# NUStatBioinfo/DegNorm

Hardware: AMD Instinct MI355X
Metric: genes/sec (20k genes x 10 samples, 5 iters) (higher is better)
Workload: dtype f64

## Files before the change

degnorm_amd/_lib.py:

```python
import ctypes
import os
import numpy as np

_HERE = os.path.dirname(os.path.abspath(__file__))
LIB_PATH = os.environ.get('DN_LIB_PATH') or os.path.join(_HERE, 'libdegnorm_amd.so')
TRACE_LEN = 48

DN_OK = 0
DN_E_INVALID, DN_E_HIP, DN_E_STATE, DN_E_UNSUPPORTED, DN_E_NO_DEVICE = -1, -2, -3, -4, -5

NMF_RANK_ONE, NMF, NMF_RATIO = 0, 1, 2
STATUS_NAMES = {0: 'ok', -1: 'ArpackError (all-zero matrix)', -2: 'empty minimum (no |K| >= 1e-5)',
                -3: 'ValueError (fewer than 2 rows or columns)', -4: 'ArpackNoConvergence (solver step cap)'}

EXIT_NAMES = ('low_cov', 'zero_sample', 'median', 'no_loop', 'refined', 'refine_fallback', 'not_found_fallback')

_lib = None


class DegnormAmdError(RuntimeError):
    pass


class Params(ctypes.Structure):
# ... 3 lines not shown


def load(build_if_missing=False):
    global _lib
    if _lib is not None:
        return _lib
    if not os.path.exists(LIB_PATH):
        if build_if_missing:
            from . import build
            build.build_library()
        else:
            raise DegnormAmdError('{0} not found: build it with `python -m degnorm_amd.build` '
                                  '(there is no CPU fallback for the NMF-OA path).'.format(LIB_PATH))
    lib = ctypes.CDLL(LIB_PATH)
    c = ctypes
    vp, i32, i64, dbl = c.c_void_p, c.c_int32, c.c_int64, c.c_double
    P = c.POINTER
    lib.dn_version.restype = c.c_char_p
    lib.dn_last_error.restype = c.c_char_p
    lib.dn_device_count.restype = c.c_int
    lib.dn_p_supported.argtypes = [c.c_int]
    lib.dn_create.argtypes = [c.c_int, P(vp)]
    lib.dn_destroy.argtypes = [vp]
    lib.dn_upload_ragged.argtypes = [vp, i64, i32, P(vp), P(i64), i32, i32, P(i64)]
    lib.dn_upload_packed.argtypes = [vp, i64, i32, P(c.c_float), P(i64)]
    lib.dn_set_downsample_hint.argtypes = [vp, i32]
    lib.dn_set_solver_step_cap.argtypes = [vp, i32]
    lib.dn_set_trace_columns.argtypes = [vp, i32]
    lib.dn_ratio_svd_sums.argtypes = [vp, P(dbl), P(dbl), P(i32)]
    lib.dn_baseline_iteration.argtypes = [vp, P(dbl), P(Params), P(i64), P(dbl), P(i32), P(i32)]
    lib.dn_fetch_estimates.argtypes = [vp, P(dbl)]
    lib.dn_outer_begin.argtypes = [vp, P(dbl), i32]
    lib.dn_init_begin.argtypes = [vp, P(dbl)]
    lib.dn_init_partials.argtypes = [vp, P(dbl)]
    lib.dn_outer_begin_scaled.argtypes = [vp, P(dbl), i32]
    lib.dn_outer_partials.argtypes = [vp, P(dbl)]
    lib.dn_outer_apply.argtypes = [vp, P(dbl), P(dbl), i32]
    lib.dn_fetch_outer.argtypes = [vp, P(dbl), P(dbl), P(dbl), P(c.c_uint8)]
    lib.dn_fetch_rows.argtypes = [vp, i64, P(i64), P(dbl), P(i32)]
    lib.dn_fetch_estimates_subset.argtypes = [vp, i64, P(i64), P(dbl)]
    lib.dn_last_kernel_ms.argtypes = [vp]
    lib.dn_last_kernel_ms.restype = dbl
    lib.dn_main_kernel_name.argtypes = [vp]
    lib.dn_main_kernel_name.restype = c.c_char_p
    lib.dn_last_span_ms.argtypes = [vp]
    lib.dn_last_span_ms.restype = dbl
    lib.dn_last_init_ms.argtypes = [vp]
    lib.dn_last_init_ms.restype = dbl
    lib.dn_init_kernel_name.argtypes = [vp]
    lib.dn_init_kernel_name.restype = c.c_char_p
    lib.dn_split_length.argtypes = [vp]
    lib.dn_split_length.restype = i32
    lib.dn_class_lengths.argtypes = [vp, i32, i32, P(i32), P(i32)]
    lib.dn_tiny_length.argtypes = [vp]
    lib.dn_tiny_length.restype = i32
    lib.dn_class_kernel_ms.argtypes = [vp, c.c_int]
    lib.dn_class_kernel_ms.restype = dbl
    lib.dn_class_kernel_name.argtypes = [vp, c.c_int]
    lib.dn_class_kernel_name.restype = c.c_char_p
    lib.dn_synchronize.argtypes = [vp]
    lib.dn_measure_copy_gbps.argtypes = [vp, i64, c.c_int]
    lib.dn_measure_copy_gbps.restype = dbl
    lib.dn_last_rowmax_ms.argtypes = [vp]
    lib.dn_last_rowmax_ms.restype = dbl
    lib.dn_measure_read_gbps.argtypes = [vp, i64, c.c_int]
    lib.dn_measure_read_gbps.restype = dbl
    lib.dn_assemble_coverage.argtypes = [c.c_int, i64, i32, P(i64), P(vp), P(vp), i64, P(i64), i64, P(i32), P(i64), P(i64), P(i32),
                                         P(c.c_float), P(dbl)]
    lib.dn_assemble_last_error.restype = c.c_char_p
    u8 = c.c_uint8
    lib.dn_read_coverage.argtypes = [c.c_int, i32, i64, P(i64), P(i64), P(u8), P(i32), i64, i64, i64, i64, i64, P(i64),
                                     i64, P(i64), P(i32), P(i32), P(i64), P(i64), P(i32), P(i64), i64, P(i64), P(i32),
                                     i64, P(i64), i64, P(i64), P(i64), i64, P(i64), P(i32), P(i64), P(i64), P(dbl)]
    lib.dn_reads_cigar_bounds.argtypes = [c.c_int, i64, P(i64), P(i64), P(u8), i32, P(i32), P(i64), P(i64)]
    lib.dn_reads_last_error.restype = c.c_char_p
    u32 = c.c_uint32
    lib.dn_bam_frame.argtypes = [P(u8), i64, i32, P(i32), P(i64), i64, P(i64), P(i64)]
    lib.dn_bam_rows_create.argtypes = [c.c_int, i32, i32, i32, P(vp)]
    lib.dn_bam_rows_destroy.argtypes = [vp]
    lib.dn_bam_rows_destroy.restype = None
    lib.dn_bam_rows_append.argtypes = [vp, P(u8), i64, P(i64), i64]
    lib.dn_bam_rows_info.argtypes = [vp, P(i64), P(i64), P(i64), P(i32)]
    lib.dn_bam_rows_keys.argtypes = [vp, i32, P(u8)]
    lib.dn_bam_rows_fetch.argtypes = [vp, P(i64), P(i64), P(i32), P(u32), P(i64), P(i32), P(u8)]
    lib.dn_bam_rows_coverage.argtypes = [vp, P(i32), P(i32), i64] + lib.dn_read_coverage.argtypes[8:]
    lib.dn_bam_cigar_bounds.argtypes = [c.c_int, i64, P(i64), P(i64), P(u32), i32, P(i32), P(i64), P(i64)]
    lib.dn_outer_partials_device.argtypes = [vp, P(vp)]
    lib.dn_comm_unique_id.argtypes = [P(c.c_uint8)]
    lib.dn_comm_create.argtypes = [vp, P(c.c_uint8), i32, i32]
    lib.dn_comm_destroy.argtypes = [vp]
    lib.dn_comm_size.argtypes = [vp]
    lib.dn_comm_size.restype = i32
    lib.dn_comm_library.restype = c.c_char_p
    lib.dn_comm_allreduce.argtypes = [vp, P(dbl), i32]
    lib.dn_init_allreduce.argtypes = [vp, P(dbl)]
    lib.dn_outer_allreduce.argtypes = [vp, P(dbl)]
    lib.dn_nmf_f64.argtypes = [vp, i64, i32, P(vp), P(i64), i32, i32, P(dbl), P(dbl), P(dbl), P(i32)]
    lib.dn_baseline_selection_f64.argtypes = [vp, i64, i32, P(vp), P(i64), P(Params), P(i64), P(dbl), P(i32), P(i32), P(dbl)]
    lib.dn_last_f64_ms.argtypes = [vp]
    lib.dn_last_f64_ms.restype = dbl
    _lib = lib
    return lib


def _check(rc):
    if rc == DN_OK:
# ... 281 lines not shown
        return Ks, Es, ests, status

    def baseline_selection_f64(self, mats, nmf_iter=100, bins=20, min_high_coverage=50, downsample_rate=1,
                               skip_baseline_selection=False, ds_start=None, want_est=False):
        keep, ptrs, lengths, p = self._f64_batch(mats)
        n = len(keep)
        prm = Params(int(nmf_iter), int(bins), int(min_high_coverage), int(downsample_rate),
                     int(bool(skip_baseline_selection)), int(bool(want_est)))
        dsp = None
        if ds_start is not None:
            ds_arr = np.ascontiguousarray(ds_start, dtype=np.int64)
            if ds_arr.shape != (n,):
                raise ValueError('ds_start must have one entry per gene')
            dsp = _p(ds_arr, ctypes.c_int64)
        rho = np.zeros((n, p))
        flags = np.zeros(n, dtype=np.int32)
        trace = np.zeros((n, TRACE_LEN), dtype=np.int32)
        est = np.zeros(p * int(lengths.sum())) if want_est else None
        _check(self.lib.dn_baseline_selection_f64(self.h, n, p, ptrs, _p(lengths, ctypes.c_int64), ctypes.byref(prm), dsp,
                                                  _p(rho, ctypes.c_double), _p(flags, ctypes.c_int32), _p(trace, ctypes.c_int32),
                                                  _p(est, ctypes.c_double) if want_est else None))
        ests = None
        if want_est:
            offs = np.concatenate([[0], np.cumsum(lengths)])
            ests = [est[p * offs[k]:p * offs[k + 1]].reshape(p, int(lengths[k])) for k in range(n)]
        return rho, flags.astype(bool), trace, ests

    def last_f64_ms(self):
        return float(self.lib.dn_last_f64_ms(self.h))

    def last_kernel_ms(self):
        return float(self.lib.dn_last_kernel_ms(self.h))

    def last_span_ms(self):
        return float(self.lib.dn_last_span_ms(self.h))

    def last_init_ms(self):
        return float(self.lib.dn_last_init_ms(self.h))

    def init_kernel_name(self):
        return self.lib.dn_init_kernel_name(self.h).decode()

    def main_kernel_name(self):
        return self.lib.dn_main_kernel_name(self.h).decode()

    def split_length(self):
        return int(self.lib.dn_split_length(self.h))

    def class_lengths(self, p, downsample_rate=1):
        a, b = ctypes.c_int32(0), ctypes.c_int32(0)
        _check(self.lib.dn_class_lengths(self.h, int(p), int(downsample_rate), ctypes.byref(a), ctypes.byref(b)))
        return int(a.value), int(b.value)

    def tiny_length(self):
        return int(self.lib.dn_tiny_length(self.h))

    def class_kernel_ms(self, cls):
        return float(self.lib.dn_class_kernel_ms(self.h, int(cls)))

    def class_kernel_name(self, cls):
        return self.lib.dn_class_kernel_name(self.h, int(cls)).decode()

    def measure_copy_gbps(self, nbytes=1 << 30, reps=5):
        return float(self.lib.dn_measure_copy_gbps(self.h, int(nbytes), int(reps)))

    def measure_read_gbps(self, nbytes=1 << 30, reps=5):
        return float(self.lib.dn_measure_read_gbps(self.h, int(nbytes), int(reps)))

    def last_rowmax_ms(self):
        return float(self.lib.dn_last_rowmax_ms(self.h))
```

degnorm_amd/csrc/dn_api.hip:

```cpp
#include "dn_kernels.hpp"
#include "dn_host.hpp"
#include "../../include/degnorm_amd.h"

#include <dlfcn.h>
#include <rccl/rccl.h>

#include <algorithm>
#include <atomic>
#include <cmath>
#include <cstdio>
#include <cstdlib>
#include <cstring>
#include <numeric>
#include <string>
#include <thread>
#include <vector>

#ifndef DN_P_MAX_TEMPLATED
#define DN_P_MAX_TEMPLATED 64
#endif
#define DN_P_2_16(X)  X(2) X(3) X(4) X(5) X(6) X(7) X(8) X(9) X(10) X(11) X(12) X(13) X(14) X(15) X(16)
#define DN_P_17_24(X) X(17) X(18) X(19) X(20) X(21) X(22) X(23) X(24)
#define DN_P_25_32(X) X(25) X(26) X(27) X(28) X(29) X(30) X(31) X(32)
#define DN_P_33_48(X) X(33) X(34) X(35) X(36) X(37) X(38) X(39) X(40) X(41) X(42) X(43) X(44) X(45) X(46) X(47) X(48)
// ... 458 lines not shown
    const int prio[dn_handle_s::NCLS] = {prio_greatest, (prio_least + prio_greatest) / 2, prio_least};
    for (int c = 0; c < dn_handle_s::NCLS; c++) {
        HIP_TRY(h->stream[c].create(hipStreamCreateWithPriority, hipStreamNonBlocking, prio[c]));
        HIP_TRY(h->ev_start[c].create(hipEventCreate));
        HIP_TRY(h->ev_end[c].create(hipEventCreate));
    }
    HIP_TRY(h->ev_ready.create(hipEventCreateWithFlags, hipEventDisableTiming));
    HIP_TRY(h->ev_i0.create(hipEventCreate));
    HIP_TRY(h->ev_i1.create(hipEventCreate));
    return DN_OK;
}

int dn_create(int device, dn_handle *out)
{
    if (!out) return fail(DN_E_INVALID, "dn_create: out is null");
    *out = nullptr;
    int ndev = 0;
    if (hipGetDeviceCount(&ndev) != hipSuccess || ndev <= 0) return fail(DN_E_NO_DEVICE, "no HIP device visible");
    if (device < 0 || device >= ndev) return fail(DN_E_INVALID, "dn_create: device index out of range");
    HIP_TRY(hipSetDevice(device));
    hipDeviceProp_t prop;
    HIP_TRY(hipGetDeviceProperties(&prop, device));
    dn_handle h = new dn_handle_s();
    h->device = device;
    h->n_cus = prop.multiProcessorCount;
    const int rc = create_streams(h);
    if (rc != DN_OK) {
        const std::string msg = g_err;
        (void) dn_destroy(h);
        return fail(rc, msg);
    }
    *out = h;
    return DN_OK;
}

int dn_destroy(dn_handle h)
{
    if (!h) return DN_OK;
    (void) hipSetDevice(h->device);
    if (h->stream[0]) (void) hipStreamSynchronize(h->stream[0]);
    (void) dn_comm_destroy(h);
    delete h;
    return DN_OK;
}

static int size_class(dn_handle h, dn_handle_s::GeneClass &C, int32_t cols)
{
    const int32_t p = h->p;
    int per_cu = C.ks->blocks_per_cu(0);
    if (per_cu < 1) per_cu = 1;
    const int units = std::max(1, C.ks->units);
    int slots = (int) std::min<int64_t>(((int64_t) C.n + units - 1) / units * units, (int64_t) per_cu * h->n_cus * units);
    const int32_t S = (cols + 63) & ~63;
    const int64_t slot_bytes = (int64_t) S * ((int64_t) p * (2 * sizeof(float) + sizeof(double)) + 3 * sizeof(double)) + (int64_t) C.ks->slot_extra_bytes;
    {
        size_t free_b = 0, total_b = 0;
        HIP_TRY(hipMemGetInfo(&free_b, &total_b));
        const int64_t budget = (int64_t) ((free_b + (C.d_ws ? (size_t) C.slot_bytes * (size_t) std::max(C.slots, 1) : 0)) / 3);
        if (slot_bytes > budget) return fail(DN_E_INVALID, "a gene is too long for the device scratch (" + std::to_string(S) + " columns)");
        slots = (int) std::max<int64_t>(units, std::min<int64_t>(slots, budget / slot_bytes / units * units));
    }
    dn::DeviceBuffer<char> ws;
    HIP_TRY(ws.alloc((size_t) slot_bytes * (size_t) std::max(slots, 1)));
    C.d_ws = std::move(ws);
    C.slots = slots; C.S = S; C.slot_bytes = slot_bytes;
    const int64_t lds_per_block = (160 * 1024) / per_cu - (int64_t) C.ks->static_lds_bytes - 256;
    const int64_t ps = p + (p & 1);
    int64_t lcols = lds_per_block > 0 ? lds_per_block / units / (8 * ps) : 0;
    lcols = std::min<int64_t>(lcols, C.S) & ~(int64_t) 1;
    C.lds_cols = (int32_t) lcols;
    C.dyn_lds = (size_t) units * (size_t) lcols * 8 * (size_t) ps;
    return DN_OK;
}

struct CoverageSource {
    const float *packed = nullptr;
    const void *const *genes = nullptr;
    int32_t is_f32 = 0, n_threads = 1;
    std::atomic<int64_t> *bad = nullptr;
};

static void pack_genes(dn_handle h, const CoverageSource &src, int64_t g0, int64_t g1, float *stage)
{
    const int32_t p = h->p;
    const int64_t base = h->goff[g0];
    std::atomic<int64_t> next(g0);
    auto work = [&]() {
        int64_t local_bad = 0;
        for (;;) {
            const int64_t a = next.fetch_add(16);
            if (a >= g1) break;
            const int64_t b = std::min(g1, a + 16);
            for (int64_t g = a; g < b; g++) {
                const int64_t cnt = (int64_t) p * h->glen[g];
                float *dst = stage + (h->goff[g] - base);
                if (src.is_f32) std::memcpy(dst, src.genes[g], sizeof(float) * (size_t) cnt);
                else {
                    const double *s = (const double *) src.genes[g];
                    for (int64_t k = 0; k < cnt; k++) { const float f = (float) s[k]; dst[k] = f; local_bad += ((double) f != s[k]); }
                }
            }
        }
        if (src.bad) *src.bad += local_bad;
    };
    const int nt = (int) std::max<int64_t>(1, std::min<int64_t>(src.n_threads, (g1 - g0 + 15) / 16));
    std::vector<std::thread> th;
    for (int t = 1; t < nt; t++) th.emplace_back(work);
// ... 901 lines not shown
    HIP_TRY(hipMemsetAsync(d_counter, 0, sizeof(int32_t) * 4, h->stream[0]));
    HIP_TRY(hipMemsetAsync(d_trace, 0, sizeof(int32_t) * (size_t) n * dn::TRACE_LEN, h->stream[0]));
    if (d_ds) HIP_TRY(hipMemcpyAsync(d_ds, ds_start, sizeof(int64_t) * (size_t) n, hipMemcpyHostToDevice, h->stream[0]));
    if (est) {
        HIP_TRY(hipMemcpyAsync(d_svoff, svoff.data(), sizeof(int64_t) * (size_t) (n + 1), hipMemcpyHostToDevice, h->stream[0]));
        HIP_TRY(hipMemcpyAsync(d_tg, tg.data(), sizeof(int32_t) * tg.size(), hipMemcpyHostToDevice, h->stream[0]));
        HIP_TRY(hipMemcpyAsync(d_tc, tc.data(), sizeof(int32_t) * tc.size(), hipMemcpyHostToDevice, h->stream[0]));
    }
    HIP_TRY(hipEventRecord(e0, h->stream[0]));
    int lrc = dn::launch_row_max_f64(d_cov, d_goff, d_glen, d_rowmax, (int) n, p,
                                     (int) std::min<int64_t>(n, (int64_t) h->n_cus * 8), h->stream[0]);
    if (lrc != 0) return fail(DN_E_HIP, std::string("k_row_max_f64 launch: ") + hipGetErrorString((hipError_t) lrc));

    dn::IterArgsF64 a;
    std::memset(&a, 0, sizeof(a));
    a.cov = d_cov; a.goff = d_goff; a.glen = d_glen; a.order = d_order; a.counter = d_counter; a.ds_start = d_ds;
    a.rowmax = d_rowmax; a.x16 = nullptr; a.ws = d_ws; a.rho = d_rho; a.flags = d_flags; a.trace = d_trace; a.kfin = d_kfin;
    a.emode = d_emode; a.svec = d_svec; a.svoff = d_svoff; a.slot_bytes = slot_bytes; a.n_genes = (int32_t) n; a.S = S;
    a.lds_cols = 0; a.T = prm->nmf_iter; a.bins = prm->bins; a.min_hc = prm->min_high_coverage; a.rate = prm->downsample_rate;
    a.skip = prm->skip_baseline_selection ? 1 : 0; a.want_est = est ? 1 : 0; a.p = p; a.max_steps = h->max_steps;
    for (int i = 0; i < dn::P_MAX; i++) { a.scale[i] = 1.0; a.inv_scale[i] = 1.0; }
    lrc = dn::launch_baseline_f64(a, grid, h->stream[0]);
    if (lrc != 0) return fail(DN_E_HIP, std::string("k_baseline_gen (float64) launch: ") + hipGetErrorString((hipError_t) lrc));
    if (est) {
        dn::EstArgsF64 e;
        std::memset(&e, 0, sizeof(e));
        e.cov = d_cov; e.goff = d_goff; e.glen = d_glen; e.kfin = d_kfin; e.emode = d_emode; e.svec = d_svec; e.svoff = d_svoff;
        e.out = d_est; e.ooff = nullptr; e.n_genes = (int32_t) n; e.p = p;
        for (int i = 0; i < dn::P_MAX; i++) e.scale[i] = 1.0;
        lrc = dn::launch_est_f64(e, d_tg, d_tc, (int) tg.size(), h->stream[0]);
        if (lrc != 0) return fail(DN_E_HIP, std::string("k_estimates_gen (float64) launch: ") + hipGetErrorString((hipError_t) lrc));
    }
    HIP_TRY(hipEventRecord(e1, h->stream[0]));
    HIP_TRY(hipMemcpyAsync(rho, d_rho, sizeof(double) * (size_t) n * p, hipMemcpyDeviceToHost, h->stream[0]));
    HIP_TRY(hipMemcpyAsync(flags, d_flags, sizeof(int32_t) * (size_t) n, hipMemcpyDeviceToHost, h->stream[0]));
    if (trace) HIP_TRY(hipMemcpyAsync(trace, d_trace, sizeof(int32_t) * (size_t) n * dn::TRACE_LEN, hipMemcpyDeviceToHost, h->stream[0]));
    if (est) HIP_TRY(hipMemcpyAsync(est, d_est, sizeof(double) * (size_t) total, hipMemcpyDeviceToHost, h->stream[0]));
    HIP_TRY(hipStreamSynchronize(h->stream[0]));
    HIP_TRY(hipEventElapsedTime(&h->last_f64_ms, e0, e1));
    return DN_OK;
}

double dn_last_f64_ms(dn_handle h) { return h ? (double) h->last_f64_ms : 0.0; }

double dn_last_kernel_ms(dn_handle h) { return h ? (double) h->last_ms : 0.0; }
double dn_last_init_ms(dn_handle h) { return h ? (double) h->last_init_ms : 0.0; }
double dn_last_span_ms(dn_handle h) { return h ? (double) h->last_span_ms : 0.0; }
double dn_last_rowmax_ms(dn_handle h) { return h ? (double) h->last_rowmax_ms : 0.0; }
const char *dn_init_kernel_name(dn_handle h) { return h ? h->init_name : ""; }
const char *dn_main_kernel_name(dn_handle h) { return (h && h->ks) ? h->ks->baseline_name : ""; }
double dn_class_kernel_ms(dn_handle h, int cls) { return (h && cls >= 0 && cls < dn_handle_s::NCLS) ? (double) h->data.cls[cls].last_ms : 0.0; }
const char *dn_class_kernel_name(dn_handle h, int cls) { return (h && cls >= 0 && cls < dn_handle_s::NCLS && h->data.cls[cls].ks && h->data.cls[cls].n > 0) ? h->data.cls[cls].ks->baseline_name : ""; }
int32_t dn_tiny_length(dn_handle h) { return h ? h->tiny_len : 0; }
int dn_class_lengths(dn_handle h, int32_t p, int32_t downsample_rate, int32_t *split_len, int32_t *tiny_len)
{
    if (!h || !split_len || !tiny_len) return fail(DN_E_INVALID, "dn_class_lengths: null argument");
    const dn::KernelSet *ks = dn::kernel_set_for(p);
    if (!ks) return fail(DN_E_UNSUPPORTED, "no kernels compiled for p = " + std::to_string(p));
    HIP_TRY(hipSetDevice(h->device));
    *split_len = 0; *tiny_len = 0;
    if (downsample_rate > 1 && p >= 8) return DN_OK;
    const dn::KernelSet *pair = nullptr;
    class_lengths(ks, p, *split_len, *tiny_len, pair);
    return DN_OK;
}
int32_t dn_split_length(dn_handle h) { return h ? h->split_len : 0; }
int dn_synchronize(dn_handle h)
{
    if (!h) return fail(DN_E_INVALID, "null handle");
    HIP_TRY(hipSetDevice(h->device));
    HIP_TRY(hipStreamSynchronize(h->stream[0]));
    return DN_OK;
}

}

__global__ __launch_bounds__(256) void k_copy4(const float4 *__restrict__ src, float4 *__restrict__ dst, size_t n4)
{
    for (size_t i = (size_t) blockIdx.x * blockDim.x + threadIdx.x; i < n4; i += (size_t) gridDim.x * blockDim.x) dst[i] = src[i];
}

__global__ __launch_bounds__(256) void k_read4(const float4 *__restrict__ src, float *__restrict__ sink, size_t n4)
{
    float acc = 0.f;
    const size_t stride = (size_t) gridDim.x * blockDim.x;
    size_t i = (size_t) blockIdx.x * blockDim.x + threadIdx.x;
    for (; i + 3 * stride < n4; i += 4 * stride) {
        const float4 a = src[i], b = src[i + stride], c = src[i + 2 * stride], d = src[i + 3 * stride];
        acc += (a.x + a.y + a.z + a.w) + (b.x + b.y + b.z + b.w) + (c.x + c.y + c.z + c.w) + (d.x + d.y + d.z + d.w);
    }
    for (; i < n4; i += stride) { const float4 a = src[i]; acc += a.x + a.y + a.z + a.w; }
    if (acc == 12345.678f) sink[0] = acc;
}

__global__ __launch_bounds__(256) void k_read8nt(const float4 *__restrict__ src, float *__restrict__ sink, size_t n4)
{
    float acc = 0.f;
    const size_t stride = (size_t) gridDim.x * blockDim.x;
    size_t i = (size_t) blockIdx.x * blockDim.x + threadIdx.x;
    for (; i + 7 * stride < n4; i += 8 * stride) {
        typedef float vf4 __attribute__((ext_vector_type(4)));
        vf4 v[8];
#pragma unroll
        for (int k = 0; k < 8; k++) v[k] = __builtin_nontemporal_load(reinterpret_cast<const vf4 *>(src + i + k * stride));
#pragma unroll
        for (int k = 0; k < 8; k++) acc += (v[k].x + v[k].y) + (v[k].z + v[k].w);
// ... 59 lines not shown
```

degnorm_amd/csrc/dn_kernels.hpp:

```cpp
#pragma once
#include <hip/hip_runtime.h>
#include <stdint.h>
#include <type_traits>
#include "dn_reduce.hpp"
#include "dn_dpp_ops.hpp"

#ifdef DN_MARKS
#define DN_MARK(name) asm volatile("; DN_MARK " name)
#else
#define DN_MARK(name)
#endif

namespace dn {

constexpr int TRACE_LEN = 48;
constexpr int MAX_BINS = 64;
constexpr int P_MAX = 64;

enum { EXIT_LOW_COV = 0, EXIT_ZERO_SAMPLE = 1, EXIT_MEDIAN = 2, EXIT_NO_LOOP = 3,
       EXIT_REFINED = 4, EXIT_REFINE_FALLBACK = 5, EXIT_NOT_FOUND_FALLBACK = 6 };
enum { LOOP_NATURAL = 0, LOOP_PERFECT = 1, LOOP_VALUE_ERROR = 2, LOOP_ZERO_ROWSUM = 3, LOOP_MIN_BINS = 4,
       LOOP_NOT_ENTERED = 5 };
enum { ST_OK = 0, ST_ARPACK = -1, ST_EMPTY_MIN = -2, ST_VALUE_ERROR = -3,
       ST_NO_CONVERGENCE = -4 };
// ... 962 lines not shown

template <int PS>
__device__ __forceinline__ void lds_col_read(const double *col, double (&a)[PS])
{
#pragma unroll
    for (int i = 0; i < PS; i += 2) { const double2 v = *reinterpret_cast<const double2 *>(col + i); a[i] = v.x; a[i + 1] = v.y; }
}
template <int PS>
__device__ __forceinline__ void lds_col_write(double *col, const double (&a)[PS])
{
#pragma unroll
    for (int i = 0; i < PS; i += 2) *reinterpret_cast<double2 *>(col + i) = make_double2(a[i], a[i + 1]);
}

typedef float dn_f4 __attribute__((ext_vector_type(4)));
typedef float dn_f2 __attribute__((ext_vector_type(2)));
typedef dn_f4 dn_f4u __attribute__((aligned(4)));
typedef dn_f2 dn_f2u __attribute__((aligned(4)));
typedef const dn_f4u __attribute__((address_space(1))) *gF4_cptr;
typedef const dn_f2u __attribute__((address_space(1))) *gF2_cptr;

template <int P>
__device__ __forceinline__ void load_x(gF_cptr Fb, int k, float (&x)[P])
{
    gF_cptr col = Fb + (size_t) k * P;
#pragma unroll
    for (int i = 0; i + 4 <= P; i += 4) {
        const dn_f4 v = *(gF4_cptr) (col + i);
        x[i] = v.x; x[i + 1] = v.y; x[i + 2] = v.z; x[i + 3] = v.w;
    }
    if constexpr ((P & 3) >= 2) {
        const dn_f2 v = *(gF2_cptr) (col + (P & ~3));
        x[P & ~3] = v.x; x[(P & ~3) + 1] = v.y;
    }
    if constexpr (P & 1) x[P - 1] = col[P - 1];
}

template <int P>
__device__ __forceinline__ void load_f(gF_cptr Fb, int k, const double (&inv)[P], double (&f)[P])
{
    float x[P];
    load_x<P>(Fb, k, x);
#pragma unroll
    for (int i = 0; i < P; i++) f[i] = (double) x[i] * inv[i];
}

template <int P, bool RAW>
__device__ __forceinline__ void pass_counts(const float (&x)[P], const double (&inv)[P], double (&f)[P])
{
#pragma unroll
    for (int i = 0; i < P; i++) f[i] = RAW ? (double) x[i] : (double) x[i] * inv[i];
}

template <int P>
__device__ __forceinline__ gdouble_ptr spill_ptr(gdouble_ptr Lg, int k)
{
    return Lg + ((size_t) (k >> 6) * (64 * P) + (size_t) (k & 63));
}

template <int P, int NT>
__device__ __forceinline__ int mg_core(gF_cptr Fb, gdouble_ptr Lg, double *lam, int n, int nL, int T,
                                       double (&u)[P], double &theta, int &steps, int maxs, bool &noconv)
{
    constexpr int W = NT / 64;
    constexpr int NG = P * (P + 1) / 2;
    constexpr int PS = P + (P & 1);
    constexpr int TR = Smem<P, NT>::MG_TR, STR = Smem<P, NT>::MG_STR;
    constexpr int NTILE = TR * (TR + 1) / 2;
    Smem<P, NT> &sm = g_sm;
    const int tid = DN_TIDX, lane = lane_id(), w = wave_id();
    const int nLe = (n < nL) ? n : nL;
    double *stage = &sm.stage[w * 16 * STR];
    double *uv = &sm.eigv[w * 128], *vv = uv + 64;
    const double *invp = g_gs.inv;
    for (int e = lane; e < 16 * STR; e += 64) stage[e] = 0.0;
    uv[lane] = lane < P ? 1.0 / sqrt((double) P) : 0.0;
    vv[lane] = 0.0;
    wave_fence();
    const int oi = lane & 15, okq = lane >> 4;
    dn_double4 acc[NTILE];

    auto feed = [&](const double (&a)[PS], bool valid) {
#pragma unroll
        for (int cq = 0; cq < 4; cq++) {
            if ((lane >> 4) == cq) {
                double *dst = stage + (lane & 15) * STR;
#pragma unroll
                for (int i = 0; i < PS; i += 2) *reinterpret_cast<double2 *>(dst + i) = make_double2(valid ? a[i] : 0.0, valid ? a[i + 1] : 0.0);
            }
            wave_fence();
#pragma unroll
            for (int g = 0; g < 4; g++) {
                double x[TR];
#pragma unroll
                for (int tr = 0; tr < TR; tr++) x[tr] = stage[(4 * g + okq) * STR + 16 * tr + oi];
                int tix = 0;
#pragma unroll
                for (int t1 = 0; t1 < TR; t1++)
#pragma unroll
                    for (int t2 = 0; t2 <= t1; t2++, tix++)
                        acc[tix] = __builtin_amdgcn_mfma_f64_16x16x4f64(x[t1], x[t2], acc[tix], 0, 0, 0);
            }
            wave_fence();
        }
    };

    const double c = 1.0 / sqrt((double) T);
    auto pass = [&](bool cold, int t) {
#pragma unroll
        for (int i = 0; i < NTILE; i++) acc[i] = dn_double4{0.0, 0.0, 0.0, 0.0};
        const int wb = w * 64;
        const int steps_l = wb < nLe ? (nLe - wb + NT - 1) / NT : 0;
        const int steps_s = nL + wb < n ? (n - nL - wb + NT - 1) / NT : 0;
#pragma clang loop unroll(disable)
        for (int j = 0; j < steps_l; j++) {
            const int k = tid + j * NT;
            const bool valid = k < nLe;
            double a[PS];
#pragma unroll
            for (int i = 0; i < PS; i++) a[i] = 0.0;
            if (valid) {
                float xr[P];
                load_x<P>(Fb, k, xr);
                if (cold) {
#pragma unroll
                    for (int i = 0; i < P; i++) a[i] = (double) xr[i] * invp[i];
                } else {
                    double al[PS], aa[P];
                    lds_col_read<PS>(lam + (size_t) k * PS, al);
#pragma unroll
                    for (int i = 0; i < P; i++) aa[i] = al[i];
                    col_update_lds<P>(xr, invp, aa, uv, c);
#pragma unroll
                    for (int i = 0; i < P; i++) a[i] = aa[i];
                }
                lds_col_write<PS>(lam + (size_t) k * PS, a);
            }
            feed(a, valid);
        }
#pragma clang loop unroll(disable)
        for (int j = 0; j < steps_s; j++) {
            const int k = nL + tid + j * NT;
            const bool valid = k < n;
            double a[PS];
#pragma unroll
            for (int i = 0; i < PS; i++) a[i] = 0.0;
            if (valid) {
                float xr[P];
                double aa[P];
                load_x<P>(Fb, k, xr);
                if (cold || t == 0) {
#pragma unroll
                    for (int i = 0; i < P; i++) aa[i] = (double) xr[i] * invp[i];
                } else {
#pragma unroll
                    for (int i = 0; i < P; i++) aa[i] = *(spill_ptr<P>(Lg, k) + i * 64);
                }
                if (!cold) {
                    col_update_lds<P>(xr, invp, aa, uv, c);
#pragma unroll
                    for (int i = 0; i < P; i++) *(spill_ptr<P>(Lg, k) + i * 64) = aa[i];
                }
#pragma unroll
                for (int i = 0; i < P; i++) a[i] = aa[i];
            }
            feed(a, valid);
        }
        {
            double *dst = (W > 1) ? sm.xw[w] : sm.tot;
            int tix = 0;
#pragma unroll
            for (int t1 = 0; t1 < TR; t1++)
#pragma unroll
                for (int t2 = 0; t2 <= t1; t2++, tix++)
#pragma unroll
                    for (int r = 0; r < 4; r++) {
                        const int row = 16 * t1 + okq + 4 * r, col = 16 * t2 + oi;
                        if (row < P && col <= row) dst[row * (row + 1) / 2 + col] = acc[tix][r];
                    }
        }
        if constexpr (W > 1) {
            dn_sync();
            for (int e = tid; e < NG; e += NT) {
                double tsum = sm.xw[0][e];
#pragma unroll
                for (int ww = 1; ww < W; ww++) tsum += sm.xw[ww][e];
                sm.tot[e] = tsum;
            }
        }
        dn_sync();
    };

    pass(true, 0);
    {
        const double tr = wave_allsum(lane < P ? sm.tot[lane * (lane + 1) / 2 + lane] : 0.0);
        if (!(tr > 0.0)) return ST_ARPACK;
    }
    { const int r = top_eig_rows_lds<P>(sm.tot, uv, vv, theta, maxs); steps += r; noconv = noconv || r > maxs; }
    bool cold_every_solve;
    {
        double um = lane < P ? uv[lane] : 1.0;
#pragma unroll
        for (int o = 32; o >= 1; o >>= 1) um = fmin(um, __shfl_xor(um, o));
        cold_every_solve = __builtin_amdgcn_readfirstlane((int) (um < WARM_START_MIN_COMPONENT)) != 0;
    }
#pragma clang loop unroll(disable)
    for (int t = 0; t < T; t++) {
        pass(false, t);
        int r;
        if (!cold_every_solve) r = top_eig_rows_lds<P>(sm.tot, uv, vv, theta, maxs);
        else {
            unsigned long long todo = P >= 64 ? ~0ull : ((1ull << P) - 1ull);
            double bul = 0.0, bth = -1.0;
            int sum = 0;
            bool capped = false;
// ... 227 lines not shown
        }
        block_sum_lds<NQ, P, NT, gram_t, false, Q * CH>(Gq, g_sm);
    });
    {
        double tr = 0.0;
#pragma unroll
        for (int i = 0; i < P; i++) tr += sm.tot[i * (i + 1) / 2 + i];
        if (!(tr > 0.0)) { if (tid == 0) g_gs.status = ST_ARPACK; dn_sync(); return; }
    }
    Solver<P> solver;
    {
        double tr = 0.0;
#pragma unroll
        for (int i = 0; i < P; i++) tr += sm.tot[i * (i + 1) / 2 + i];
        solver.cold(tr, u);
    }
    {
        const int r = SAFE ? solve_by_blocks<P>(solver, sm.tot, Smem<P, NT>::ZSLOT, u, theta, maxs)
                           : solver.run(sm.tot, Smem<P, NT>::ZSLOT, u, theta, T == 0, maxs, true);
        steps += r; noconv = noconv || r > maxs;
    }
    const double c = 1.0 / sqrt((double) T);
    auto pass_u = [&]() {
        if constexpr (RAW) {
            const int k = Solver<P>::row_of_lane() < P ? Solver<P>::row_of_lane() : P - 1;
            const double vt = solver.iterate_of_row() * g_gs.inv[k], vh = solver.iterate_of_row() * g_gs.scl[k];
#pragma unroll
            for (int i = 0; i < P; i++) { ud[i] = Solver<P>::bcast_component(vt, i); ur[i] = Solver<P>::bcast_component(vh, i); }
        } else {
#pragma unroll
            for (int i = 0; i < P; i++) { u[i] = uniform(u[i]); ud[i] = u[i]; ur[i] = u[i]; }
        }
    };
    pass_u();

    static_for<0, RT>([&](auto rc) {
        constexpr int R = decltype(rc)::value;
        const int k = tid + R * NT;
        if (k < n) {
            float xf[P];
            double f[P];
            load_x<P>(Fb, k, xf);
            pass_counts<P, RAW>(xf, inv, f);
            rt_write<P, CS * R>(f);
            if constexpr (X16) rt_write_counts<P, CS * R + 2 * P>(xf);
        }
    });
    for (int k = NR + tid; k < nLe; k += NT) {
        double f[P], a[PS];
        { float xf[P]; load_x<P>(Fb, k, xf); pass_counts<P, RAW>(xf, inv, f); }
#pragma unroll
        for (int i = 0; i < PS; i++) a[i] = i < P ? f[i] : 0.0;
        lds_col_write<PS>(lam + (size_t) (k - NR) * PS, a);
    }
#ifdef DN_STAMP
    stamp[3] += __builtin_amdgcn_s_memtime() - t_cold0;
#endif
    constexpr bool G0 = FULL && ONCHIP && SW == 1;
    constexpr bool SQ = Solver<P>::SQUARE && SW == 1 && !SAFE;
#pragma clang loop unroll(disable)
    for (int t = 0; t < T; t++) {
        DN_MARK("iter_begin");
        if constexpr (!G0) {
#pragma unroll
            for (int i = 0; i < CH; i++) G[i] = 0.0;
        }
        DN_MARK("zeroed");
        { DN_T0();
        const int dir = (t & 1) ? -1 : 1;

        auto reg_tier = [&]() {
            if constexpr (RT > 0 && X16) {
                auto column = [&](auto rc) {
                    constexpr int R = decltype(rc)::value;
                    double f[P], a[P];
                    rt_read_counts<P, CS * R + 2 * P>(f);
                    if constexpr (!RAW) {
#pragma unroll
                        for (int i = 0; i < P; i++) f[i] *= inv[i];
                    }
                    rt_read<P, CS * R>(a);
                    col_update<P>(f, a, ud, ur, c);
                    if constexpr (G0 && R == 0) gram_set_range<P, 0, CH>(G, a); else gram_add_range<P, 0, CH>(G, a);
                    rt_write<P, CS * R>(a);
                };
                if constexpr (FULL) {
                    static_for<0, RT>([&](auto rc) { column(rc); __builtin_amdgcn_sched_barrier(0); });
                } else {
                    static_for<0, RT>([&](auto rc) {
                        constexpr int R = decltype(rc)::value;
                        if (tid + R * NT < n) column(rc);
                    });
                }
            } else if constexpr (RT > 0) {
                float xq[P];
                if (tid < n) load_x<P>(Fb, tid, xq);
                static_for<0, RT>([&](auto rc) {
                    constexpr int R = decltype(rc)::value;
                    const int k = tid + R * NT;
                    if (k < n) {
                        double f[P], a[P];
                        pass_counts<P, RAW>(xq, inv, f);
                        if constexpr (R + 1 < RT) load_x<P>(Fb, k + NT < n ? k + NT : k, xq);
                        rt_read<P, CS * R>(a);
                        col_update<P>(f, a, ud, ur, c);
                        gram_add_range<P, 0, CH>(G, a);
                        rt_write<P, CS * R>(a);
                    }
                });
            }
        };
        auto lds_tier = [&]() {
            const int first = NR + tid;
            const int cnt = first < nLe ? (nLe - first + NT - 1) / NT : 0;
            const int step = dir * NT;
            int k = dir > 0 ? first : first + (cnt - 1) * NT;
            float xq[P];
            if (cnt > 0) load_x<P>(Fb, k, xq);
#pragma clang loop unroll(disable)
            for (int j = 0; j < cnt; j++, k += step) {
                double f[P], a[PS];
                lds_col_read<PS>(lam + (size_t) (k - NR) * PS, a);
                pass_counts<P, RAW>(xq, inv, f);
                load_x<P>(Fb, j + 1 < cnt ? k + step : k, xq);
                double aa[P];
#pragma unroll
                for (int i = 0; i < P; i++) aa[i] = a[i];
                col_update<P>(f, aa, ud, ur, c);
                gram_add_range<P, 0, CH>(G, aa);
#pragma unroll
                for (int i = 0; i < P; i++) a[i] = aa[i];
                lds_col_write<PS>(lam + (size_t) (k - NR) * PS, a);
            }
        };
        auto spill_tier = [&]() {
            if constexpr (ONCHIP) return;
            const int first = kS0 + tid;
            const int cnt = first < n ? (n - first + NT - 1) / NT : 0;
            const int step = dir * NT;
            int k = dir > 0 ? first : first + (cnt - 1) * NT;
            float xn[P];
            double an[P];
            if (cnt > 0) {
                int kq = k;
                asm volatile("" : "+v"(kq));
                load_x<P>(Fb, kq, xn);
                if (t > 0) {
#pragma unroll
                    for (int i = 0; i < P; i++) an[i] = *(spill_ptr<P>(Lg, kq) + i * 64);
                }
            }
#pragma clang loop unroll(disable)
            for (int j = 0; j < cnt; j++, k += step) {
                double f[P], a[P];
                pass_counts<P, RAW>(xn, inv, f);
#pragma unroll
                for (int i = 0; i < P; i++) a[i] = t > 0 ? an[i] : f[i];
                if (j + 1 < cnt) {
                    load_x<P>(Fb, k + step, xn);
                    if (t > 0) {
#pragma unroll
                        for (int i = 0; i < P; i++) an[i] = *(spill_ptr<P>(Lg, k + step) + i * 64);
                    }
                }
                col_update<P>(f, a, ud, ur, c);
                gram_add_range<P, 0, CH>(G, a);
#pragma unroll
                for (int i = 0; i < P; i++) *(spill_ptr<P>(Lg, k) + i * 64) = a[i];
            }
        };
#if defined(DN_STAMP) && defined(DN_EXP_TIER)
#define DN_TIER(id, call) do { if (DN_EXP_TIER == id) { const long long tt_ = __builtin_amdgcn_s_memtime(); call; stamp[0] += __builtin_amdgcn_s_memtime() - tt_; } else { call; } } while (0)
#else
#define DN_TIER(id, call) call
#endif
        if constexpr (G0) { DN_MARK("reg_tier"); DN_TIER(1, reg_tier()); DN_MARK("lds_tier"); DN_TIER(2, lds_tier()); }
        else if (dir > 0) { DN_MARK("reg_tier"); DN_TIER(1, reg_tier()); DN_MARK("lds_tier"); DN_TIER(2, lds_tier()); DN_MARK("spill_tier"); DN_TIER(3, spill_tier()); }
        else { DN_MARK("spill_tier_b"); DN_TIER(3, spill_tier()); DN_MARK("lds_tier_b"); DN_TIER(2, lds_tier()); DN_MARK("reg_tier_b"); DN_TIER(1, reg_tier()); }
        DN_MARK("pass_end");
#if !(defined(DN_STAMP) && defined(DN_EXP_TIER))
        DN_T1(0);
#endif
        }
        { DN_T0(); block_sum_lds<CH, P, NT, gram_t, Solver<P>::SHIFTED, 0, RAW, SQ>(G, sm, solver.shift(), solver.scale(), t & 1); DN_T1(1); }
        DN_MARK("reduced");
        static_for<1, SW>([&](auto qc) {
            constexpr int Q = decltype(qc)::value;
            constexpr int NQ = (NG - Q * CH) < CH ? (NG - Q * CH) : CH;
            gram_t Gq[NQ];
#pragma unroll
            for (int i = 0; i < NQ; i++) Gq[i] = 0.0;
            static_assert(SW == 1 || RT == 0, "the later sweeps do not read the register tier");
#pragma clang loop unroll(disable)
            for (int k = NR + tid; k < nLe; k += NT) {
                double a[PS], aa[P];
                lds_col_read<PS>(lam + (size_t) (k - NR) * PS, a);
#pragma unroll
                for (int i = 0; i < P; i++) aa[i] = a[i];
                gram_add_range<P, Q * CH, NQ>(Gq, aa);
            }
#pragma clang loop unroll(disable)
            for (int k = kS0 + tid; k < n; k += NT) {
                double aa[P];
#pragma unroll
                for (int i = 0; i < P; i++) aa[i] = *(spill_ptr<P>(Lg, k) + i * 64);
                gram_add_range<P, Q * CH, NQ>(Gq, aa);
            }
            block_sum_lds<NQ, P, NT, gram_t, Solver<P>::SHIFTED, Q * CH>(Gq, g_sm, solver.shift());
        });
        { DN_T0();
        double u_unused[P];
        double (&us_)[P] = RAW ? u_unused : u;
        const int r = SAFE ? solve_by_blocks<P>(solver, sm.tot, Smem<P, NT>::ZSLOT, us_, theta, maxs)
                           : solver.template run<SQ>(sm.tot, Smem<P, NT>::ZSLOT, us_, theta, t == T - 1, maxs, false,
                                                     sm.sq + wave_id() * Smem<P, NT>::SQ_LEN);
        steps += r; noconv = noconv || r > maxs;
        pass_u();
        DN_MARK("solved");
        DN_T1(2);
        }
    }
    if constexpr (SQ && NT > 64) dn_sync();
    if constexpr (RAW) {
#pragma unroll
        for (int i = 0; i < P; i++) u[i] = Solver<P>::bcast_component(solver.iterate_of_row(), i);
    }
    }

#ifdef DN_STAMP
    const long long t_fin0 = __builtin_amdgcn_s_memtime();
#endif
    double invf[P];
#pragma unroll
    for (int i = 0; i < P; i++) invf[i] = RAW ? uniform(g_gs.inv[i]) : inv[i];
    double acc[2 * P + 1];
#pragma unroll
    for (int i = 0; i < 2 * P + 1; i++) acc[i] = 0.0;
    auto fin = [&](int k, const double (&f)[P], const double (&l_)[P]) {
        double s, r, l0[P];
#pragma unroll
        for (int i = 0; i < P; i++) l0[i] = RAW ? l_[i] * invf[i] : l_[i];
        col_final<P>(f, l0, u, first, acc, s, r);
        rs[k] = r;
        if (first) sv[k] = s;
    };
    static_for<0, RT>([&](auto rc) {
        constexpr int R = decltype(rc)::value;
        const int k = tid + R * NT;
        if (k < n) {
            double f[P], l[P];
            if constexpr (X16) {
                rt_read_counts<P, CS * R + 2 * P>(f);
#pragma unroll
                for (int i = 0; i < P; i++) f[i] *= invf[i];
            } else load_f<P>(Fb, k, invf, f);
            rt_read<P, CS * R>(l);
            fin(k, f, l);
        }
    });
    float xqf[P];
    if (NR + tid < n) load_x<P>(Fb, NR + tid, xqf);
#pragma clang loop unroll(disable)
    for (int k = NR + tid; k < n; k += NT) {
        double f[P], l[P];
#pragma unroll
        for (int i = 0; i < P; i++) f[i] = (double) xqf[i] * invf[i];
        load_x<P>(Fb, k + NT < n ? k + NT : k, xqf);
        if (k < nLe) {
            double al[PS];
            lds_col_read<PS>(lam + (size_t) (k - NR) * PS, al);
#pragma unroll
            for (int i = 0; i < P; i++) l[i] = al[i];
        } else {
#pragma unroll
            for (int i = 0; i < P; i++) l[i] = *(spill_ptr<P>(Lg, k) + i * 64);
        }
        fin(k, f, l);
    }
    block_sum_lds<2 * P + 1, P, NT, double>(acc, sm);
    for (int e = tid; e < 2 * P + 1; e += NT) g_gs.sums[e] = sm.tot[e];
    if (tid == 0) {
#pragma unroll
        for (int i = 0; i < P; i++) g_gs.u[i] = u[i];
        g_gs.theta = theta;
        g_gs.steps += steps;
        g_gs.status = noconv ? ST_NO_CONVERGENCE : ST_OK;
#ifdef DN_STAMP
        g_gs.stamp[0] += stamp[0]; g_gs.stamp[1] += stamp[1]; g_gs.stamp[2] += stamp[2];
        g_gs.stamp[4] += __builtin_amdgcn_s_memtime() - t_fin0; g_gs.stamp[5] += stamp[3];
#endif
    }
    dn_sync();
}

template <int P, int NT, bool SAFE = false>
__device__ __attribute__((noinline)) void nmf_call(const float *Fb_, double *Lg_, double *rs_, double *sv_, double *rtsave_,
                                                   int n, int S, int nL, int T, int first_i, int x16_i)
{
    constexpr int NSAVE = DN_REG_TIER ? rt_regs_used<P>() : 0;
    int *rtsave = reinterpret_cast<int *>(uniform_ptr(rtsave_));
#ifdef DN_STAMP
    const long long t_call0 = __builtin_amdgcn_s_memtime();
#endif
    const int n_u = __builtin_amdgcn_readfirstlane(n);
    const int need = DN_REG_TIER ? ((n_u + NT - 1) / NT) * rt_col_regs<P, true>() : 0;
    rt_save<NSAVE, NT>(rtsave, need);
    if constexpr (SAFE) {
        nmf_body<P, NT, false, false, false, true>(Fb_, Lg_, rs_, sv_, n, S, nL, T, first_i);
    } else if (DN_REG_TIER && __builtin_amdgcn_readfirstlane(x16_i) != 0) {
        constexpr bool X = DN_REG_TIER != 0;
        const int nL_u = __builtin_amdgcn_readfirstlane(nL);
        if (X && n_u >= rt_cols<P, X>() * NT && n_u <= rt_cols<P, X>() * NT + nL_u)
            nmf_body<P, NT, X, X, X>(Fb_, Lg_, rs_, sv_, n, S, nL, T, first_i);
        else if (X && n_u >= rt_cols<P, X>() * NT) nmf_body<P, NT, X, X>(Fb_, Lg_, rs_, sv_, n, S, nL, T, first_i);
        else nmf_body<P, NT, X, false>(Fb_, Lg_, rs_, sv_, n, S, nL, T, first_i);
    } else nmf_body<P, NT, false>(Fb_, Lg_, rs_, sv_, n, S, nL, T, first_i);
    rt_restore<NSAVE, NT>(rtsave, need);
#ifdef DN_STAMP
    if (DN_TIDX == 0) g_gs.stamp[3] += __builtin_amdgcn_s_memtime() - t_call0;
#endif
}


template <int P> __device__ __forceinline__ double lds_max(const double *v)
{ double m = v[0];
#pragma unroll
  for (int i = 1; i < P; i++) { const double t = v[i]; m = t > m ? t : m; } return m; }
template <int P> __device__ __forceinline__ double lds_min(const double *v)
{ double m = v[0];
#pragma unroll
  for (int i = 1; i < P; i++) { const double t = v[i]; m = t < m ? t : m; } return m; }

template <int P, int NT>
__global__ __launch_bounds__(NT * DN_UNITS, DN_KERNEL_WAVES) void k_baseline(IterArgs A)
{
    constexpr int W = NT / 64;
    Smem<P, NT> &sm = g_sm;
    GeneState<P> &gs = g_gs;
    const int tid = DN_TIDX, lane = lane_id(), w = wave_id();
    const int S = A.S;
    const int nL = A.lds_cols;
    char *slot = A.ws + ((size_t) blockIdx.x * DN_UNITS + DN_UNIT) * A.slot_bytes;
    float *Fs = reinterpret_cast<float *>(slot);
    float *Fb = Fs + (size_t) P * S;
    double *Lg = reinterpret_cast<double *>(Fb + (size_t) P * S);
    double *sv = Lg + (size_t) P * S;
    double *rs = sv + S;
    double *rtsave = rs + 2 * (size_t) S;
    DN_RT_CLAIM();
    if (tid < P) { gs.inv[tid] = A.inv_scale[tid]; gs.scl[tid] = 1.0 / A.inv_scale[tid]; }
    if (tid == 0) gs.max_steps = A.max_steps > 0 ? A.max_steps : EIG_MAX_STEPS_DEFAULT;
    if constexpr (P <= 16) { for (int t = tid; t < W * Smem<P, NT>::SQ_LEN; t += NT) sm.sq[t] = 0.0; }
    for (int t = tid; t < Smem<P, NT>::NX; t += NT) {
        bool diag = false;
        int ra = 0, rb = 0;
#pragma unroll
        for (int i = 0; i < P; i++) {
            diag = diag || (t == i * (i + 1) / 2 + i);
            if (t >= i * (i + 1) / 2) { ra = i; rb = t - i * (i + 1) / 2; }
        }
        if constexpr (P <= 16) sm.sqi[t] = (t < P * (P + 1) / 2) ? (ra * Smem<P, NT>::SQ_STR + rb) | ((rb * Smem<P, NT>::SQ_STR + ra) << 16) : 0;
        if constexpr (raw_units<P>())
            sm.dsel[t] = (t < P * (P + 1) / 2) ? (diag ? -1.0 : 1.0) * A.inv_scale[ra] * A.inv_scale[rb < P ? rb : 0] : 0.0;
        else sm.dsel[t] = diag ? 1.0 : 0.0;
        if (t == Smem<P, NT>::ZSLOT) sm.tot[t] = 0.0;
    }

    for (;;) {
        if (tid == 0) sm.gene = atomicAdd(A.counter, 1);
        dn_sync();
        const int q = sm.gene;
        dn_sync();
        if (q >= A.n_genes) break;
        const int g = A.order[q];
        const int L = A.glen[g];
        const float *x = A.cov + A.goff[g];

        int n0 = 0, n_calls = 0, n_drops = 0, exit_code = EXIT_LOW_COV, loop_reason = LOOP_NOT_ENTERED;
        int status = ST_OK, flag = 0, emode = EM_INPUT;
        long long sum_cols = 0;
#ifdef DN_STAMP
        const long long t_gene0 = __builtin_amdgcn_s_memtime();
        long long t_ret = 0, t_book = 0;
#endif
        int32_t *tr = A.trace + (size_t) g * TRACE_LEN;
        if (tid < P) { gs.rho[tid] = 0.0; gs.K[tid] = 0.0; gs.us[tid] = 0.0; }
        if (tid == 0) { gs.steps = 0; gs.stamp[0] = gs.stamp[1] = gs.stamp[2] = gs.stamp[3] = gs.stamp[4] = gs.stamp[5] = 0; }

        double thr;
        int x16;
        {
            const float *rmx = A.rowmax + (size_t) g * P;
            double gmax = (double) rmx[0] / A.scale[0];
#pragma unroll
            for (int i = 1; i < P; i++) { const double v = (double) rmx[i] / A.scale[i]; gmax = v > gmax ? v : gmax; }
            thr = 0.1 * gmax;
            x16 = A.x16[g];
        }

// ... 419 lines not shown
```

include/degnorm_amd.h:

```cpp
#ifndef DEGNORM_AMD_H
#define DEGNORM_AMD_H

#include <stdint.h>

#ifdef __cplusplus
extern "C" {
#endif

#define DN_OK                 0
#define DN_E_INVALID         -1
#define DN_E_HIP             -2
#define DN_E_STATE           -3
#define DN_E_UNSUPPORTED     -4
#define DN_E_NO_DEVICE       -5

#define DN_TRACE_LEN          48

typedef struct dn_handle_s *dn_handle;

typedef struct {
    int32_t nmf_iter;
    int32_t bins;
    int32_t min_high_coverage;
    int32_t downsample_rate;
// ... 66 lines not shown

#define DN_READS_MAX_SEG      32
int  dn_read_coverage(int device, int32_t paired, int64_t n_rows, const int64_t *pos, const int64_t *cigar_off,
                      const uint8_t *cigar, const int32_t *pair_id, int64_t n_pair_ids,
                      int64_t chrom_len, int64_t keep_lo, int64_t keep_hi,
                      int64_t n_exon, const int64_t *exon_iv,
                      int64_t n_groups, const int64_t *group_iv, const int32_t *group_gene_off,
                      const int32_t *ol_gene, const int64_t *ol_gene_start0, const int64_t *ol_cov_off,
                      const int32_t *ol_exon_off, const int64_t *ol_exon_bounds,
                      int64_t n_iso, const int64_t *iso_iv, const int32_t *iso_gene,
                      int64_t n_iso_union, const int64_t *iso_union,
                      int64_t n_genes, int64_t *counts, int64_t *ol_cov,
                      int64_t csr_cap, int64_t *nnz, int32_t *csr_idx, int64_t *csr_val,
                      int64_t *n_isolated_reads, double *device_ms);
int  dn_reads_cigar_bounds(int device, int64_t n, const int64_t *pos, const int64_t *cigar_off, const uint8_t *cigar,
                           int32_t max_seg, int32_t *nseg, int64_t *bounds, int64_t *end_pos);
const char *dn_reads_last_error(void);

typedef struct dn_bam_rows_s *dn_bam_rows;
int  dn_bam_frame(const uint8_t *buf, int64_t n_bytes, int32_t tid, int32_t *last_pos, int64_t *rec_off, int64_t cap,
                  int64_t *n_rec, int64_t *consumed);
int  dn_bam_rows_create(int device, int32_t tid, int32_t unique_alignment, int32_t paired, dn_bam_rows *out);
void dn_bam_rows_destroy(dn_bam_rows h);
int  dn_bam_rows_append(dn_bam_rows h, const uint8_t *window, int64_t n_bytes, const int64_t *rec_off, int64_t n_rec);
int  dn_bam_rows_info(dn_bam_rows h, int64_t *n_rows, int64_t *n_ops, int64_t *n_name_bytes, int32_t *max_key_len);
int  dn_bam_rows_keys(dn_bam_rows h, int32_t width, uint8_t *keys);
int  dn_bam_rows_fetch(dn_bam_rows h, int64_t *pos, int64_t *op_beg, int32_t *n_op, uint32_t *ops, int64_t *name_beg,
                       int32_t *name_len, uint8_t *names);
int  dn_bam_rows_coverage(dn_bam_rows h, const int32_t *order, const int32_t *pair_id, int64_t n_pair_ids,
                          int64_t chrom_len, int64_t keep_lo, int64_t keep_hi,
                          int64_t n_exon, const int64_t *exon_iv,
                          int64_t n_groups, const int64_t *group_iv, const int32_t *group_gene_off,
                          const int32_t *ol_gene, const int64_t *ol_gene_start0, const int64_t *ol_cov_off,
                          const int32_t *ol_exon_off, const int64_t *ol_exon_bounds,
                          int64_t n_iso, const int64_t *iso_iv, const int32_t *iso_gene,
                          int64_t n_iso_union, const int64_t *iso_union,
                          int64_t n_genes, int64_t *counts, int64_t *ol_cov,
                          int64_t csr_cap, int64_t *nnz, int32_t *csr_idx, int64_t *csr_val,
                          int64_t *n_isolated_reads, double *device_ms);
int  dn_bam_cigar_bounds(int device, int64_t n, const int64_t *pos, const int64_t *op_off, const uint32_t *ops,
                         int32_t max_seg, int32_t *nseg, int64_t *bounds, int64_t *end_pos);

double dn_last_kernel_ms(dn_handle h);
const char *dn_main_kernel_name(dn_handle h);
double dn_last_init_ms(dn_handle h);
double dn_last_rowmax_ms(dn_handle h);
const char *dn_init_kernel_name(dn_handle h);
int32_t dn_split_length(dn_handle h);
int  dn_class_lengths(dn_handle h, int32_t p, int32_t downsample_rate, int32_t *split_len, int32_t *tiny_len);
int32_t dn_tiny_length(dn_handle h);
double dn_class_kernel_ms(dn_handle h, int cls);
double dn_last_span_ms(dn_handle h);
const char *dn_class_kernel_name(dn_handle h, int cls);
int  dn_synchronize(dn_handle h);
double dn_measure_copy_gbps(dn_handle h, int64_t bytes, int reps);
double dn_measure_read_gbps(dn_handle h, int64_t bytes, int reps);

#ifdef __cplusplus
}
#endif
#endif
```

Baseline: 15220.

## Pair-interleave global spill columns for 128-bit loads and prefill spill tier

Changes the global-memory spill layout for per-column lambda values from one double per row-stride to pairs of doubles (padded to an even P), so each column is read and written with 16-byte vector accesses through a shared base pointer with constant offsets. The cold init pass now writes initial spill values, which lets the spill tier loop drop its t==0 branching and always prefetch the next column with clamped indices, restructured as a do-while. It also adds a diagnostic API that reports register/LDS tier column counts. The cost is padding memory for odd P and an extra initial write pass over spilled columns.

```diff
diff --git a/degnorm_amd/_lib.py b/degnorm_amd/_lib.py
--- a/degnorm_amd/_lib.py
+++ b/degnorm_amd/_lib.py
@@ -79,6 +79,7 @@
     lib.dn_split_length.argtypes = [vp]
     lib.dn_split_length.restype = i32
     lib.dn_class_lengths.argtypes = [vp, i32, i32, P(i32), P(i32)]
+    lib.dn_class_tier_cols.argtypes = [vp, c.c_int, P(i32), P(i32)]
     lib.dn_tiny_length.argtypes = [vp]
     lib.dn_tiny_length.restype = i32
     lib.dn_class_kernel_ms.argtypes = [vp, c.c_int]
@@ -466,6 +467,11 @@
         _check(self.lib.dn_class_lengths(self.h, int(p), int(downsample_rate), ctypes.byref(a), ctypes.byref(b)))
         return int(a.value), int(b.value)
 
+    def class_tier_cols(self, cls):
+        a, b = ctypes.c_int32(0), ctypes.c_int32(0)
+        _check(self.lib.dn_class_tier_cols(self.h, int(cls), ctypes.byref(a), ctypes.byref(b)))
+        return int(a.value), int(b.value)
+
     def tiny_length(self):
         return int(self.lib.dn_tiny_length(self.h))
 
diff --git a/degnorm_amd/csrc/dn_api.hip b/degnorm_amd/csrc/dn_api.hip
--- a/degnorm_amd/csrc/dn_api.hip
+++ b/degnorm_amd/csrc/dn_api.hip
@@ -534,7 +534,8 @@
     const int units = std::max(1, C.ks->units);
     int slots = (int) std::min<int64_t>(((int64_t) C.n + units - 1) / units * units, (int64_t) per_cu * h->n_cus * units);
     const int32_t S = (cols + 63) & ~63;
-    const int64_t slot_bytes = (int64_t) S * ((int64_t) p * (2 * sizeof(float) + sizeof(double)) + 3 * sizeof(double)) + (int64_t) C.ks->slot_extra_bytes;
+    const int64_t slot_bytes = (int64_t) S * ((int64_t) p * 2 * sizeof(float) + (int64_t) (p + (p & 1)) * sizeof(double) + 3 * sizeof(double)) +
+                               (int64_t) C.ks->slot_extra_bytes;
     {
         size_t free_b = 0, total_b = 0;
         HIP_TRY(hipMemGetInfo(&free_b, &total_b));
@@ -1542,6 +1543,15 @@
 double dn_class_kernel_ms(dn_handle h, int cls) { return (h && cls >= 0 && cls < dn_handle_s::NCLS) ? (double) h->data.cls[cls].last_ms : 0.0; }
 const char *dn_class_kernel_name(dn_handle h, int cls) { return (h && cls >= 0 && cls < dn_handle_s::NCLS && h->data.cls[cls].ks && h->data.cls[cls].n > 0) ? h->data.cls[cls].ks->baseline_name : ""; }
 int32_t dn_tiny_length(dn_handle h) { return h ? h->tiny_len : 0; }
+int dn_class_tier_cols(dn_handle h, int cls, int32_t *reg_cols, int32_t *lds_cols)
+{
+    if (!h || cls < 0 || cls >= dn_handle_s::NCLS || !reg_cols || !lds_cols) return fail(DN_E_INVALID, "dn_class_tier_cols: bad argument");
+    const auto &C = h->data.cls[cls];
+    const bool live = C.ks && C.n > 0;
+    *reg_cols = live ? C.ks->reg_tier_cols : 0;
+    *lds_cols = live ? C.lds_cols : 0;
+    return DN_OK;
+}
 int dn_class_lengths(dn_handle h, int32_t p, int32_t downsample_rate, int32_t *split_len, int32_t *tiny_len)
 {
     if (!h || !split_len || !tiny_len) return fail(DN_E_INVALID, "dn_class_lengths: null argument");
diff --git a/degnorm_amd/csrc/dn_kernels.hpp b/degnorm_amd/csrc/dn_kernels.hpp
--- a/degnorm_amd/csrc/dn_kernels.hpp
+++ b/degnorm_amd/csrc/dn_kernels.hpp
@@ -1038,10 +1038,32 @@
     for (int i = 0; i < P; i++) f[i] = RAW ? (double) x[i] : (double) x[i] * inv[i];
 }
 
+typedef double dn_d2 __attribute__((ext_vector_type(2)));
+typedef dn_d2 __attribute__((address_space(1))) *gd2_ptr;
+template <int P> constexpr int spill_mid() { return (P + (P & 1)) / 4; }
 template <int P>
-__device__ __forceinline__ gdouble_ptr spill_ptr(gdouble_ptr Lg, int k)
-{
-    return Lg + ((size_t) (k >> 6) * (64 * P) + (size_t) (k & 63));
+__device__ __forceinline__ gd2_ptr spill_col(gdouble_ptr Lg, int k)
+{
+    constexpr int PS = P + (P & 1);
+    gd2_ptr col = (gd2_ptr) (Lg + ((size_t) (k >> 6) * (64 * PS) + (size_t) (k & 63) * 2)) + spill_mid<P>() * 64;
+    asm volatile("" : "+v"(col));
+    return col;
+}
+template <int P>
+__device__ __forceinline__ void spill_col_read(gd2_ptr col, double (&a)[P])
+{
+#pragma unroll
+    for (int q = 0; q < (P + 1) / 2; q++) {
+        const dn_d2 v = col[(q - spill_mid<P>()) * 64];
+        a[2 * q] = v.x;
+        if (2 * q + 1 < P) a[2 * q + 1] = v.y;
+    }
+}
+template <int P>
+__device__ __forceinline__ void spill_col_write(gd2_ptr col, const double (&a)[P])
+{
+#pragma unroll
+    for (int q = 0; q < (P + 1) / 2; q++) col[(q - spill_mid<P>()) * 64] = dn_d2{a[2 * q], 2 * q + 1 < P ? a[2 * q + 1 < P ? 2 * q + 1 : 2 * q] : 0.0};
 }
 
 template <int P, int NT>
@@ -1135,18 +1157,15 @@
                 float xr[P];
                 double aa[P];
                 load_x<P>(Fb, k, xr);
-                if (cold || t == 0) {
+                const gd2_ptr col = spill_col<P>(Lg, k);
+                if (cold) {
 #pragma unroll
                     for (int i = 0; i < P; i++) aa[i] = (double) xr[i] * invp[i];
                 } else {
-#pragma unroll
-                    for (int i = 0; i < P; i++) aa[i] = *(spill_ptr<P>(Lg, k) + i * 64);
+                    spill_col_read<P>(col, aa);
+                    col_update_lds<P>(xr, invp, aa, uv, c);
                 }
-                if (!cold) {
-                    col_update_lds<P>(xr, invp, aa, uv, c);
-#pragma unroll
-                    for (int i = 0; i < P; i++) *(spill_ptr<P>(Lg, k) + i * 64) = aa[i];
-                }
+                spill_col_write<P>(col, aa);
 #pragma unroll
                 for (int i = 0; i < P; i++) a[i] = aa[i];
             }
@@ -1480,6 +1499,13 @@
 #pragma unroll
         for (int i = 0; i < PS; i++) a[i] = i < P ? f[i] : 0.0;
         lds_col_write<PS>(lam + (size_t) (k - NR) * PS, a);
+    }
+    if constexpr (!ONCHIP) {
+        for (int k = kS0 + tid; k < n; k += NT) {
+            double f[P];
+            { float xf[P]; load_x<P>(Fb, k, xf); pass_counts<P, RAW>(xf, inv, f); }
+            spill_col_write<P>(spill_col<P>(Lg, k), f);
+        }
     }
 #ifdef DN_STAMP
     stamp[3] += __builtin_amdgcn_s_memtime() - t_cold0;
@@ -1563,39 +1589,34 @@
         };
         auto spill_tier = [&]() {
             if constexpr (ONCHIP) return;
-            const int first = kS0 + tid;
-            const int cnt = first < n ? (n - first + NT - 1) / NT : 0;
+            int tq = tid;
+            asm volatile("" : "+v"(tq));
+            const int first = kS0 + tq;
+            if (first >= n) return;
             const int step = dir * NT;
-            int k = dir > 0 ? first : first + (cnt - 1) * NT;
+            const int last = first + (n - 1 - first) / NT * NT;
+            int k = dir > 0 ? first : last;
+            const int kend = dir > 0 ? last : first;
             float xn[P];
             double an[P];
-            if (cnt > 0) {
-                int kq = k;
-                asm volatile("" : "+v"(kq));
-                load_x<P>(Fb, kq, xn);
-                if (t > 0) {
-#pragma unroll
-                    for (int i = 0; i < P; i++) an[i] = *(spill_ptr<P>(Lg, kq) + i * 64);
-                }
-            }
+            load_x<P>(Fb, k, xn);
+            spill_col_read<P>(spill_col<P>(Lg, k), an);
+            bool more;
 #pragma clang loop unroll(disable)
-            for (int j = 0; j < cnt; j++, k += step) {
+            do {
                 double f[P], a[P];
                 pass_counts<P, RAW>(xn, inv, f);
 #pragma unroll
-                for (int i = 0; i < P; i++) a[i] = t > 0 ? an[i] : f[i];
-                if (j + 1 < cnt) {
-                    load_x<P>(Fb, k + step, xn);
-                    if (t > 0) {
-#pragma unroll
-                        for (int i = 0; i < P; i++) an[i] = *(spill_ptr<P>(Lg, k + step) + i * 64);
-                    }
-                }
+                for (int i = 0; i < P; i++) a[i] = an[i];
+                const int kn = dir > 0 ? min(k + step, kend) : max(k + step, kend);
+                load_x<P>(Fb, kn, xn);
+                spill_col_read<P>(spill_col<P>(Lg, kn), an);
                 col_update<P>(f, a, ud, ur, c);
                 gram_add_range<P, 0, CH>(G, a);
-#pragma unroll
-                for (int i = 0; i < P; i++) *(spill_ptr<P>(Lg, k) + i * 64) = a[i];
-            }
+                spill_col_write<P>(spill_col<P>(Lg, k), a);
+                more = k != kend;
+                k += step;
+            } while (more);
         };
 #if defined(DN_STAMP) && defined(DN_EXP_TIER)
 #define DN_TIER(id, call) do { if (DN_EXP_TIER == id) { const long long tt_ = __builtin_amdgcn_s_memtime(); call; stamp[0] += __builtin_amdgcn_s_memtime() - tt_; } else { call; } } while (0)
@@ -1630,8 +1651,7 @@
 #pragma clang loop unroll(disable)
             for (int k = kS0 + tid; k < n; k += NT) {
                 double aa[P];
-#pragma unroll
-                for (int i = 0; i < P; i++) aa[i] = *(spill_ptr<P>(Lg, k) + i * 64);
+                spill_col_read<P>(spill_col<P>(Lg, k), aa);
                 gram_add_range<P, Q * CH, NQ>(Gq, aa);
             }
             block_sum_lds<NQ, P, NT, gram_t, Solver<P>::SHIFTED, Q * CH>(Gq, g_sm, solver.shift());
@@ -1699,10 +1719,7 @@
             lds_col_read<PS>(lam + (size_t) (k - NR) * PS, al);
 #pragma unroll
             for (int i = 0; i < P; i++) l[i] = al[i];
-        } else {
-#pragma unroll
-            for (int i = 0; i < P; i++) l[i] = *(spill_ptr<P>(Lg, k) + i * 64);
-        }
+        } else spill_col_read<P>(spill_col<P>(Lg, k), l);
         fin(k, f, l);
     }
     block_sum_lds<2 * P + 1, P, NT, double>(acc, sm);
@@ -1772,7 +1789,7 @@
     float *Fs = reinterpret_cast<float *>(slot);
     float *Fb = Fs + (size_t) P * S;
     double *Lg = reinterpret_cast<double *>(Fb + (size_t) P * S);
-    double *sv = Lg + (size_t) P * S;
+    double *sv = Lg + (size_t) (P + (P & 1)) * S;
     double *rs = sv + S;
     double *rtsave = rs + 2 * (size_t) S;
     DN_RT_CLAIM();
diff --git a/include/degnorm_amd.h b/include/degnorm_amd.h
--- a/include/degnorm_amd.h
+++ b/include/degnorm_amd.h
@@ -142,6 +142,7 @@
 double dn_class_kernel_ms(dn_handle h, int cls);
 double dn_last_span_ms(dn_handle h);
 const char *dn_class_kernel_name(dn_handle h, int cls);
+int  dn_class_tier_cols(dn_handle h, int cls, int32_t *reg_cols, int32_t *lds_cols);
 int  dn_synchronize(dn_handle h);
 double dn_measure_copy_gbps(dn_handle h, int64_t bytes, int reps);
 double dn_measure_read_gbps(dn_handle h, int64_t bytes, int reps);
```

Result: faster. 15440 (median of 6 runs) (+1.4%).
